# LUP-LuftbildUmweltPlanung/UNet

Hardware: AMD Instinct MI355X
Metric: 512x512 tiles/sec fwd+bwd (4-ch->5-class U-Net) (higher is better)
Workload: dtype f32

## Files before the change

### include/unet_hip.h

```cpp
#ifndef UNET_HIP_H
#define UNET_HIP_H

#include <stddef.h>
#include <stdint.h>

#ifdef __cplusplus
extern "C" {
#endif

#define UNET_OK 0
#define UNET_E_BADARG (-1)
#define UNET_E_UNSUPPORTED (-2)
#define UNET_E_HIP (-3)

#define UNET_ABI_VERSION 8

int unet_abi_version(void);
const char* unet_last_error(void);

#define UNET_F32 0
#define UNET_BF16 1
typedef uint16_t unet_bf16;

typedef struct {
    int conv_splitk;
    int mfma_shape;
    int f32_big_tile;
    int bf16_big_tile;
    int t256_tiles_per_wg;
    int t256_sliver;
    int conv1x1_gemm;
    int wgrad_mfma_shape;
    int wgrad_bf16_k4;
    int wgrad_1x1;
    int wgrad_narrow;
    int plan_batch;
    int wgrad_wgs;
    int conv_smallcin;
    int conv_head1x1;
} unet_tuning;
void unet_tuning_default(unet_tuning* t);


#define UNET_CONV_RELU 1
#define UNET_CONV_MASK 4

#define UNET_CONV_FWD 0
#define UNET_CONV_DGRAD 1

typedef struct {
    const float* x; int x_cs, x_co;
    const float* wp;
    const float* bias;
    const float* res; int res_cs, res_co;
    const float* mask; int mask_cs, mask_co;
    float* y; int y_cs, y_co;
    int N, IH, IW, Cin;
    int OH, OW, Cout;
    int ks, stride;
    int kind, flags;
    float* colsum;
    float* colsumsq;
    int cout_begin, cout_count;
    long long wp_img_stride;
    int dtype;
    int y_f32;
    float* splitk_ws;
    size_t splitk_ws_floats;
    const unet_tuning* tuning;
    int pixel_shuffle;
    const void* ps_tail;
    int ps_tail_cs, ps_tail_co;
    int ps_tail_c, ps_tail_at;
} unet_conv_desc;

int unet_conv2d_colsum_rows(const unet_conv_desc* d);
int unet_conv2d(const unet_conv_desc* d, void* stream);
size_t unet_conv2d_splitk_workspace(const unet_conv_desc* d);
int unet_conv2d_variant(const unet_conv_desc* d);
size_t unet_pack_weights_size(int Cout, int Cin, int ks, int mode);
int unet_pack_weights(const float* w, float* wp, int Cout, int Cin, int ks, int mode, void* stream);
int unet_pack_weights_strided(const float* w, long long so, long long sr, float* wp, int O, int R, void* stream);
size_t unet_pack_weights_size_bf16(int Cout, int Cin, int ks, int mode);
int unet_pack_weights_bf16(const float* w, unet_bf16* wp, int Cout, int Cin, int ks, int mode, void* stream);
typedef struct {
    const float* w;
    void* wp;
    int Cout, Cin, ks, mode;
    const float* out_scale;
} unet_pack_job;
size_t unet_pack_batch_table_bytes(int njobs);
int unet_pack_batch_build(const unet_pack_job* jobs, int njobs, int dtype, void* table_host, unsigned* total_blocks);
int unet_pack_batch_run(const void* table_dev, int njobs, unsigned total_blocks, int dtype, void* stream);
typedef struct {
    const float* x; int x_cs, x_co;
    const float* dy; int dy_cs, dy_co;
    float* dw;
    float* dbias;
    int N, IH, IW, Cin, OH, OW, Cout, ks, stride;
    float* workspace; size_t workspace_floats;
    int accumulate;
    int dtype;
    const unet_tuning* tuning;
} unet_wgrad_desc;
size_t unet_conv2d_wgrad_workspace(const unet_wgrad_desc* d);
int unet_conv2d_wgrad_dma(const unet_wgrad_desc* d);
int unet_conv2d_wgrad(const unet_wgrad_desc* d, void* stream);

int unet_bn_stats_rows(long long P);
int unet_bn_stats(const float* x, int x_cs, int x_co, long long P, int C, float* partial, void* stream);
int unet_bn_finalize(const float* psum, const float* psumsq, int rows, long long count, int C,
                     const float* gamma, const float* beta, float* running_mean, float* running_var,
                     float momentum, float eps,
                     float* scale, float* shift, float* save_mean, float* save_invstd, long long* batches_tracked, void* stream);
int unet_bn_eval_coeffs(const float* gamma, const float* beta, const float* running_mean, const float* running_var,
                        float eps, int C, float* scale, float* shift, void* stream);
int unet_affine_act(const float* x, int x_cs, int x_co, const float* scale, const float* shift,
                    const float* x2, int x2_cs, int x2_co, const float* scale2, const float* shift2,
                    float* y, int y_cs, int y_co, long long P, int C, int relu, void* stream);
int unet_bn_bwd_reduce(const float* dout, int d_cs, int d_co, const float* out, int o_cs, int o_co,
                       const float* x, int x_cs, int x_co, const float* mean, const float* invstd,
                       long long P, int C, float* partial, void* stream);
int unet_bn_bwd_finalize(const float* partial, int rows, long long count, int C,
                         float* dgamma, float* dbeta, float* c1, float* c2, void* stream);
int unet_bn_bwd_apply(const float* dout, int d_cs, int d_co, const float* out, int o_cs, int o_co,
                      const float* x, int x_cs, int x_co, const float* mean, const float* invstd,
                      const float* gamma, const float* c1, const float* c2,
                      float* dx, int dx_cs, int dx_co, float* gout, int g_cs, int g_co, int g_accumulate,
                      long long P, int C, void* stream);

int unet_maxpool3x3s2(const float* x, int x_cs, int x_co, float* y, int y_cs, int y_co, uint8_t* idx,
                      int N, int IH, int IW, int C, int OH, int OW, void* stream);
int unet_maxpool3x3s2_bwd(const float* dy, int dy_cs, int dy_co, const uint8_t* idx, float* dx, int dx_cs, int dx_co,
                          int N, int IH, int IW, int C, int OH, int OW, int accumulate, void* stream);
int unet_avgpool2_ceil(const float* x, int x_cs, int x_co, float* y, int y_cs, int y_co,
                       int N, int IH, int IW, int C, int OH, int OW, void* stream);
int unet_avgpool2_ceil_bwd(const float* dy, int dy_cs, int dy_co, float* dx, int dx_cs, int dx_co,
                           int N, int IH, int IW, int C, int OH, int OW, int accumulate, void* stream);

int unet_shuffle_blur(const float* yc, int yc_cs, int yc_co, float* X, int X_cs, int X_co,
                      int N, int h, int w, int Cu, int do_blur, void* stream);
int unet_shuffle_blur_bwd(const float* dX, int dX_cs, int dX_co, const float* yc, int yc_cs, int yc_co,
                          float* dyc, int dyc_cs, int dyc_co, int N, int h, int w, int Cu, int do_blur, void* stream);
int unet_shuffle_bwd_xmask(const float* dX, int dX_cs, int dX_co, const float* X, int X_cs, int X_co,
                           float* dyc, int dyc_cs, int dyc_co, int N, int h, int w, int Cu, void* stream);
int unet_resize_nearest(const float* x, int x_cs, int x_co, float* y, int y_cs, int y_co,
                        int N, int IH, int IW, int OH, int OW, int C, void* stream);
int unet_resize_nearest_bwd(const float* dy, int dy_cs, int dy_co, float* dx, int dx_cs, int dx_co,
                            int N, int IH, int IW, int OH, int OW, int C, void* stream);
int unet_nchw_to_nhwc(const float* x, float* y, int y_cs, int y_co, int N, int C, int H, int W, void* stream);
int unet_nhwc_to_nchw(const float* x, int x_cs, int x_co, float* y, int N, int C, int H, int W, void* stream);
int unet_copy_slice(const float* x, int x_cs, int x_co, float* y, int y_cs, int y_co, long long P, int C,
                    int accumulate, void* stream);
int unet_relu_mask(const float* g, int g_cs, int g_co, const float* ref, int r_cs, int r_co,
                   float* y, int y_cs, int y_co, long long P, int C, void* stream);
int unet_colsum(const float* x, int x_cs, int x_co, long long P, int C, float* out, float* workspace, void* stream);
size_t unet_colsum_workspace(long long P, int C);
int unet_dot(const float* x, int x_cs, int x_co, const float* y, int y_cs, int y_co, long long P, int C, float* out,
             float* workspace, void* stream);

size_t unet_ce_workspace(long long P);
int unet_ce_fwd(const float* z, int z_cs, int z_co, const int64_t* target, const float* weight, long long P, int C,
// ... 308 lines not shown
```

### unet_amd/csrc/conv1x1.hip

```cpp
#include "conv_common.h"

namespace {

typedef float f32x4 __attribute__((ext_vector_type(4)));
typedef __bf16 bf16x8 __attribute__((ext_vector_type(8)));
typedef __bf16 bf16x4 __attribute__((ext_vector_type(4)));
typedef unsigned short u16;

struct G1Args {
    const char* x; const char* wp; const float* bias; const char* res; const char* mask; char* y;
    int x_cs, x_co, res_cs, res_co, mask_cs, mask_co, y_cs, y_co;
    long long P;
    int nchunks, coutPad, n_base, n_end, Cout, relu, y_f32, ntn;
    long long ntiles;
    int ps, nf, H, W;
    const char* tail; int tail_cs, tail_co, tail_q, tail_at;
};

template <typename T, bool STAGED>
__global__ __launch_bounds__(256, 2) void conv1x1_gemm_kernel(const G1Args a) {
    constexpr int EB = (int)sizeof(T), KCB = 64;
    constexpr int MT = STAGED ? 8 : 4, NT = 4, TPIX = MT * 32, ROWB = 96, BUFB = TPIX * ROWB;
    extern __shared__ __attribute__((aligned(16))) char lds[];
    const int tid = threadIdx.x, lane = tid & 63, wave = __builtin_amdgcn_readfirstlane(tid >> 6);
    const int wm = wave >> 1, wn = wave & 1, l15 = lane & 15, kq = lane >> 4;
    const long long per_xcd = (long long)(gridDim.x >> 3);
    const long long wg = (long long)(blockIdx.x & 7) * per_xcd + (long long)(blockIdx.x >> 3);
    if (wg >= a.ntiles) return;
    const int nb = (int)(wg % a.ntn);
    const long long pt = wg / a.ntn;
    const long long p0 = pt * TPIX + wm * (TPIX / 2);
    const int c0 = a.n_base + nb * 128;

    const char* xp[MT];
#pragma unroll
    for (int m = 0; m < MT; ++m) {
        long long p = p0 + m * 16 + l15;
        p = p < a.P ? p : a.P - 1;
        xp[m] = a.x + ((size_t)p * a.x_cs + a.x_co) * EB + 16 * kq;
    }
    const char* wl = a.wp + ((size_t)(c0 + wn * 16 + l15) * KCB + 16 * kq);
    const size_t slab = (size_t)a.coutPad * KCB;
    int nv = 0;
#pragma unroll
    for (int n = 0; n < NT; ++n) nv += (c0 + (2 * n + wn) * 16 < a.n_end) ? 1 : 0;
    nv = __builtin_amdgcn_readfirstlane(nv);

    f32x4 acc[MT][NT];
#pragma unroll
    for (int m = 0; m < MT; ++m)
#pragma unroll
        for (int n = 0; n < NT; ++n) acc[m][n] = (f32x4){0.f, 0.f, 0.f, 0.f};

    auto mma = [&](const f32x4 (&xs)[MT], const f32x4 (&ws)[NT]) {
#pragma unroll
        for (int n = 0; n < NT; ++n) {
            if (n < nv) {
                if constexpr (EB == 2) {
                    const bf16x8 wv = __builtin_bit_cast(bf16x8, ws[n]);
#pragma unroll
                    for (int m = 0; m < MT; ++m)
                        acc[m][n] = __builtin_amdgcn_mfma_f32_16x16x32_bf16(wv, __builtin_bit_cast(bf16x8, xs[m]), acc[m][n], 0, 0, 0);
                } else {
#pragma unroll
                    for (int kk = 0; kk < 4; ++kk)
#pragma unroll
                        for (int m = 0; m < MT; ++m) acc[m][n] = __builtin_amdgcn_mfma_f32_16x16x4f32(ws[n][kk], xs[m][kk], acc[m][n], 0, 0, 0);
                }
            }
        }
    };
    const int last = a.nchunks - 1;
    if constexpr (!STAGED) {
        f32x4 xa[MT], wa[NT], xb[MT], wb[NT];
        auto load = [&](f32x4 (&xs)[MT], f32x4 (&ws)[NT], int c) {
#pragma unroll
            for (int m = 0; m < MT; ++m) xs[m] = *reinterpret_cast<const f32x4*>(xp[m] + (size_t)c * KCB);
#pragma unroll
            for (int n = 0; n < NT; ++n) ws[n] = *reinterpret_cast<const f32x4*>(wl + (size_t)c * slab + (size_t)n * 2048);
        };
        load(xa, wa, 0);
        for (int c = 0; c < a.nchunks; c += 2) {
            load(xb, wb, c + 1 < last ? c + 1 : last);
            mma(xa, wa);
            load(xa, wa, c + 2 < last ? c + 2 : last);
            if (c + 1 < a.nchunks) mma(xb, wb);
        }
    } else {
        const char* sp[4];
        unsigned so[4];
#pragma unroll
        for (int it = 0; it < 4; ++it) {
            const int e = tid + 256 * it, pe = e >> 2, q = e & 3;
            long long p = pt * TPIX + pe;
            p = p < a.P ? p : a.P - 1;
            sp[it] = a.x + ((size_t)p * a.x_cs + a.x_co) * EB + 16 * q;
            so[it] = (unsigned)(pe * ROWB + 16 * q);
        }
        const unsigned rbase = (unsigned)((wm * (TPIX / 2) + l15) * ROWB + 16 * kq);
// ... 25 lines not shown
            gload(wa, c + 2 < last ? c + 2 : last);
            if (c + 1 < a.nchunks) stage(wb, 1);
            sstore(0);
            __syncthreads();
        }
    }

    const T* resb = reinterpret_cast<const T*>(a.res);
    const T* maskb = reinterpret_cast<const T*>(a.mask);
    auto ld4 = [](const T* p_) -> f32x4 {
        if constexpr (EB == 2) {
            const uint2 u = *reinterpret_cast<const uint2*>(p_);
            return (f32x4){__uint_as_float(u.x << 16), __uint_as_float(u.x & 0xffff0000u), __uint_as_float(u.y << 16), __uint_as_float(u.y & 0xffff0000u)};
        } else return *reinterpret_cast<const f32x4*>(p_);
    };
    f32x4 bv[NT];
    int c4s[NT];
#pragma unroll
    for (int n = 0; n < NT; ++n) {
        const int c4 = c0 + (2 * n + wn) * 16 + 4 * kq;
        c4s[n] = c4;
        bv[n] = (f32x4){0.f, 0.f, 0.f, 0.f};
        if (a.bias != nullptr && n < nv && c4 < a.n_end) {
            if (a.ps) {
                const int ij = c4 / a.nf, c = c4 - ij * a.nf;
#pragma unroll
                for (int q = 0; q < 4; ++q) bv[n][q] = a.bias[4 * (c + q) + ij];
            } else {
#pragma unroll
                for (int q = 0; q < 4; ++q) bv[n][q] = (c4 + q < a.Cout) ? a.bias[c4 + q] : 0.f;
            }
        }
    }
#pragma unroll
    for (int m = 0; m < MT; ++m) {
        const long long p = p0 + m * 16 + l15;
        if (p >= a.P) continue;
        long long pimg = 0;
        int ph = 0, pw = 0;
        if (a.ps) {
            pimg = p / ((long long)a.H * a.W);
            const int rem = (int)(p - pimg * a.H * a.W);
            ph = rem / a.W; pw = rem - ph * a.W;
        }
#pragma unroll
        for (int n = 0; n < NT; ++n) {
            if (n >= nv) continue;
            const int c4 = c4s[n];
            if (c4 >= a.n_end) continue;
            f32x4 v = acc[m][n] + bv[n];
            if (resb != nullptr) v += ld4(resb + (size_t)p * a.res_cs + a.res_co + c4);
            if (a.relu) {
#pragma unroll
                for (int q = 0; q < 4; ++q) v[q] = fmaxf(v[q], 0.f);
            }
            if (maskb != nullptr) {
                const f32x4 mv = ld4(maskb + (size_t)p * a.mask_cs + a.mask_co + c4);
#pragma unroll
                for (int q = 0; q < 4; ++q) v[q] = mv[q] > 0.f ? v[q] : 0.f;
            }
            size_t yo = (size_t)p * a.y_cs + a.y_co + c4;
            if (a.ps) {
                const int ij = c4 / a.nf, c = c4 - ij * a.nf;
                yo = ((size_t)(pimg * 2 * a.H + 2 * ph + (ij >> 1)) * (2 * a.W) + 2 * pw + (ij & 1)) * a.y_cs + a.y_co + c;
            }
            if (EB == 4 || a.y_f32) *reinterpret_cast<f32x4*>(reinterpret_cast<float*>(a.y) + yo) = v;
            else {
                const bf16x4 o = {(__bf16)v[0], (__bf16)v[1], (__bf16)v[2], (__bf16)v[3]};
                *reinterpret_cast<uint2*>(reinterpret_cast<u16*>(a.y) + yo) = __builtin_bit_cast(uint2, o);
            }
            if (a.ps && a.tail != nullptr && c4 % a.nf == a.nf - 4) {
                const size_t op = (yo - (size_t)a.y_co - (size_t)(a.nf - 4)) / (size_t)a.y_cs;
                const char* src = a.tail + ((size_t)op * a.tail_cs + a.tail_co) * EB;
                char* dst = a.y + ((size_t)op * a.y_cs + a.tail_at) * EB;
                for (int t = 0; t < a.tail_q; ++t) {
                    if constexpr (EB == 4) *reinterpret_cast<f32x4*>(dst + 16 * t) = *reinterpret_cast<const f32x4*>(src + 16 * t);
                    else *reinterpret_cast<uint2*>(dst + 8 * t) = *reinterpret_cast<const uint2*>(src + 8 * t);
                }
            }
        }
    }
}


struct HeadArgs {
    const char* x; const char* wp; const float* bias; char* y;
    int x_cs, x_co, y_cs, y_co;
    long long P;
    int Cin, Cout, coutPad, relu, y_f32;
};

template <typename T, int NCH, int MT>
__global__ __launch_bounds__(256) void conv1x1_head_kernel(const HeadArgs a) {
    constexpr int EB = (int)sizeof(T), KC = 64 / EB, VEC = 16 / EB;
    const int lane = threadIdx.x & 63, l15 = lane & 15, kq = lane >> 4;
    const int nch = (a.Cin + KC - 1) / KC, tail = a.Cin % KC;
    const int cin_v = (a.Cin + VEC - 1) / VEC * VEC;
    f32x4 w[NCH];
#pragma unroll
    for (int c = 0; c < NCH; ++c) {
        w[c] = (f32x4){0.f, 0.f, 0.f, 0.f};
        if (c < nch) w[c] = *reinterpret_cast<const f32x4*>(a.wp + ((size_t)(c * a.coutPad + l15) * KC) * EB + 16 * kq);
    }
    float bv[4];
#pragma unroll
    for (int r = 0; r < 4; ++r) bv[r] = (a.bias != nullptr && 4 * kq + r < a.Cout) ? a.bias[4 * kq + r] : 0.f;
    const long long nwaves = (long long)gridDim.x * 4, wave0 = (long long)blockIdx.x * 4 + (threadIdx.x >> 6);
    constexpr int WP = 16 * MT;
    auto ldx = [](const char* q) { return *reinterpret_cast<const f32x4*>(q); };
    for (long long g = wave0; g * WP < a.P; g += nwaves) {
        f32x4 xs[MT][NCH];
        const char* xp[MT];
#pragma unroll
        for (int m = 0; m < MT; ++m) {
            long long p = g * WP + m * 16 + l15;
            p = p < a.P ? p : a.P - 1;
            xp[m] = a.x + ((size_t)p * a.x_cs + a.x_co) * EB;
#pragma unroll
            for (int c = 0; c < NCH; ++c) {
                xs[m][c] = (f32x4){0.f, 0.f, 0.f, 0.f};
                if constexpr (EB == 4) {
                    if (c < nch && !(tail != 0 && c == nch - 1)) xs[m][c] = ldx(xp[m] + (size_t)(c * KC + 4 * kq) * EB);
                    else if (c == nch - 1 && tail != 0) {
#pragma unroll
                        for (int kk = 0; kk < 4; ++kk)
                            if (kq + 4 * kk < tail) xs[m][c][kk] = *reinterpret_cast<const float*>(xp[m] + (size_t)(c * KC + kq + 4 * kk) * EB);
                    }
                } else {
                    if (c < nch && c * KC + VEC * kq < cin_v) xs[m][c] = ldx(xp[m] + (size_t)(c * KC + VEC * kq) * EB);
                }
            }
        }
        f32x4 acc[MT];
#pragma unroll
        for (int m = 0; m < MT; ++m) acc[m] = (f32x4){0.f, 0.f, 0.f, 0.f};
#pragma unroll
        for (int c = 0; c < NCH; ++c) {
            if (c < nch) {
                if constexpr (EB == 2) {
#pragma unroll
                    for (int m = 0; m < MT; ++m)
                        acc[m] = __builtin_amdgcn_mfma_f32_16x16x32_bf16(__builtin_bit_cast(bf16x8, w[c]), __builtin_bit_cast(bf16x8, xs[m][c]), acc[m], 0, 0, 0);
                } else {
                    const int steps = (tail != 0 && c == nch - 1) ? (tail + 3) / 4 : 4;
#pragma unroll
                    for (int kk = 0; kk < 4; ++kk)
                        if (kk < steps) {
#pragma unroll
                            for (int m = 0; m < MT; ++m) acc[m] = __builtin_amdgcn_mfma_f32_16x16x4f32(w[c][kk], xs[m][c][kk], acc[m], 0, 0, 0);
                        }
                }
            }
        }
        if (4 * kq < a.Cout) {
            const int nr = a.Cout - 4 * kq;
#pragma unroll
            for (int m = 0; m < MT; ++m) {
                const long long p = g * WP + m * 16 + l15;
                if (p >= a.P) continue;
                f32x4 v = acc[m];
#pragma unroll
                for (int r = 0; r < 4; ++r) {
                    v[r] += bv[r];
                    if (a.relu) v[r] = fmaxf(v[r], 0.f);
                }
                if (EB == 4 || a.y_f32) {
                    float* yo = reinterpret_cast<float*>(a.y) + (size_t)p * a.y_cs + a.y_co + 4 * kq;
                    if (nr >= 4) *reinterpret_cast<f32x4*>(yo) = v;
                    else {
#pragma unroll
                        for (int r = 0; r < 3; ++r) if (r < nr) yo[r] = v[r];
                    }
                } else {
                    __bf16* yo = reinterpret_cast<__bf16*>(a.y) + (size_t)p * a.y_cs + a.y_co + 4 * kq;
                    if (nr >= 4) *reinterpret_cast<bf16x4*>(yo) = (bf16x4){(__bf16)v[0], (__bf16)v[1], (__bf16)v[2], (__bf16)v[3]};
                    else {
#pragma unroll
                        for (int r = 0; r < 3; ++r) if (r < nr) yo[r] = (__bf16)v[r];
                    }
                }
            }
        }
    }
}
}

namespace unetconv {

static bool shape_ok(const unet_conv_desc* d) {
    if (d->ks != 1 || d->stride != 1 || d->wp_img_stride != 0 || d->colsum != nullptr || d->colsumsq != nullptr) return false;
    const int kct = d->dtype == UNET_BF16 ? 32 : 16;
    if (d->Cin < kct || d->Cin % kct != 0) return false;
    if (d->cout_begin % 128 != 0) return false;
    const int cols = d->cout_count ? d->cout_count : d->Cout;
    if (cols % 4 != 0 && d->cout_begin + cols != d->Cout) return false;
    const int pb = tuning_of(d->tuning).plan_batch;
    const long long P = (long long)(pb > 0 ? pb : d->N) * d->OH * d->OW;
    return ((P + 127) / 128) * ((cols + 127) / 128) >= 256;
}
static int form_of(const unet_conv_desc* d) {
    const int mode = tuning_of(d->tuning).conv1x1_gemm;
    if (d->pixel_shuffle) return mode == 1 ? 1 : 2;
    if (mode < 0) return 0;
    if (mode == 0) return d->dtype == UNET_BF16 ? 2 : 0;
    return mode == 1 ? 1 : 2;
}
bool conv_gemm1x1_applies(const unet_conv_desc* d) { return form_of(d) != 0 && shape_ok(d); }

int conv_gemm1x1_ps_check(const unet_conv_desc* d) {
    UNET_CHECK_ARG(d->x && d->wp && d->y && unet::aligned16(d->x) && unet::aligned16(d->wp) && unet::aligned16(d->y), "conv pixel_shuffle: null / unaligned tensor pointer");
    UNET_CHECK_ARG(d->dtype == UNET_F32 || d->dtype == UNET_BF16, "conv: unknown dtype %d", d->dtype);
    const int vec = d->dtype == UNET_BF16 ? 8 : 4;
    UNET_CHECK_ARG(d->ks == 1 && d->stride == 1 && d->kind == UNET_CONV_FWD && d->N > 0 && d->IH > 0 && d->IW > 0 && d->OH == d->IH && d->OW == d->IW && d->Cin > 0 && d->Cout > 0,
                   "conv pixel_shuffle: a 1x1 / stride-1 forward convolution");
    UNET_CHECK_ARG(d->Cout % 64 == 0, "conv pixel_shuffle: Cout = 4 nf with nf a multiple of 16 (got %d)", d->Cout);
    UNET_CHECK_ARG(unet::slice_ok_v(d->x_cs, d->x_co, d->Cin, vec), "conv pixel_shuffle: bad x slice");
    UNET_CHECK_ARG(unet::slice_ok_v(d->y_cs, d->y_co, d->Cout / 4, 4), "conv pixel_shuffle: bad y slice (Cout / 4 channels of a [N, 2 OH, 2 OW] tensor)");
    UNET_CHECK_ARG((d->flags & ~(UNET_CONV_RELU | UNET_CONV_MASK)) == 0, "conv pixel_shuffle: unknown flag bits 0x%x", d->flags);
    UNET_CHECK_ARG(d->bias == nullptr || (((uintptr_t)d->bias) & 3) == 0, "conv pixel_shuffle: bias must be a float pointer");
    UNET_CHECK_ARG(d->res == nullptr && !(d->flags & UNET_CONV_MASK) && d->colsum == nullptr && d->colsumsq == nullptr && d->cout_begin == 0 &&
                   d->cout_count == 0 && d->wp_img_stride == 0, "conv pixel_shuffle: no residual / mask / column sums / channel range / per-image filters");
    UNET_CHECK_ARG((long long)d->N * d->OH * d->OW * 4 < (1ll << 31), "conv pixel_shuffle: more than 2^31 output pixels");
    if (d->ps_tail != nullptr) {
        const int tq = unet::roundup(d->ps_tail_c, 4);
        UNET_CHECK_ARG(unet::aligned16(d->ps_tail) && d->ps_tail_c > 0 && d->ps_tail_cs > 0 && d->ps_tail_cs % 4 == 0 && d->ps_tail_co >= 0 && d->ps_tail_co % 4 == 0 &&
                       d->ps_tail_co + tq <= d->ps_tail_cs, "conv pixel_shuffle: bad ps_tail slice (whole quads: cs, co multiples of 4, co + roundup(c, 4) <= cs)");
        UNET_CHECK_ARG(d->ps_tail_at % 4 == 0 && d->ps_tail_at >= d->y_co + d->Cout / 4 && d->ps_tail_at + tq <= d->y_cs && !(d->dtype == UNET_BF16 && d->y_f32),
                       "conv pixel_shuffle: ps_tail_at must be a multiple of 4 behind the shuffled channels with ps_tail_at + roundup(ps_tail_c, 4) <= y_cs");
    }
    if (!shape_ok(d)) {
        unet::set_error("conv pixel_shuffle: only conv1x1_gemm_kernel stores pixel-shuffled (whole reduction chunks, >= 256 blocks of 128 x 128); "
                        "ask unet_conv2d_variant first and keep conv + unet_shuffle_blur otherwise");
        return UNET_E_UNSUPPORTED;
    }
    return UNET_OK;
}

int conv_gemm1x1(const unet_conv_desc* d, hipStream_t st) {
    G1Args a;
    const bool bf = d->dtype == UNET_BF16;
    const int kct = bf ? 32 : 16;
    a.x = (const char*)d->x; a.wp = (const char*)d->wp; a.bias = d->bias; a.res = (const char*)d->res;
    a.mask = (d->flags & UNET_CONV_MASK) ? (const char*)d->mask : nullptr; a.y = (char*)d->y;
    a.x_cs = d->x_cs; a.x_co = d->x_co; a.res_cs = d->res_cs; a.res_co = d->res_co; a.mask_cs = d->mask_cs; a.mask_co = d->mask_co;
    a.y_cs = d->y_cs; a.y_co = d->y_co;
    a.P = (long long)d->N * d->OH * d->OW;
    a.nchunks = d->Cin / kct;
    a.coutPad = unet::roundup(d->Cout, 128);
    a.n_base = d->cout_begin;
    a.n_end = d->cout_begin + (d->cout_count ? d->cout_count : d->Cout);
    a.Cout = d->Cout;
    a.relu = (d->flags & UNET_CONV_RELU) ? 1 : 0;
    a.y_f32 = bf ? d->y_f32 : 1;
    a.tail = d->pixel_shuffle ? (const char*)d->ps_tail : nullptr;
    a.tail_cs = d->ps_tail_cs; a.tail_co = d->ps_tail_co; a.tail_q = unet::roundup(d->ps_tail_c, 4) / 4; a.tail_at = d->ps_tail_at;
    const bool staged = form_of(d) == 2;
    const int tpix = staged ? 256 : 128;
    a.ntn = unet::cdiv(a.n_end - a.n_base, 128);
    a.ntiles = ((a.P + tpix - 1) / tpix) * a.ntn;
    a.ps = d->pixel_shuffle ? 1 : 0; a.nf = d->Cout / 4; a.H = d->OH; a.W = d->OW;
    UNET_CHECK_ARG(a.ntiles < (1ll << 31) - 8, "conv 1x1: grid too large");
    const unsigned grid = (unsigned)((a.ntiles + 7) / 8 * 8);
    if (staged) {
        if (bf) hipLaunchKernelGGL((conv1x1_gemm_kernel<unsigned short, true>), dim3(grid), dim3(256), 2 * 256 * 96, st, a);
        else hipLaunchKernelGGL((conv1x1_gemm_kernel<float, true>), dim3(grid), dim3(256), 2 * 256 * 96, st, a);
    } else {
        if (bf) hipLaunchKernelGGL((conv1x1_gemm_kernel<unsigned short, false>), dim3(grid), dim3(256), 0, st, a);
        else hipLaunchKernelGGL((conv1x1_gemm_kernel<float, false>), dim3(grid), dim3(256), 0, st, a);
    }
    UNET_CHECK_LAUNCH();
    return UNET_OK;
}


bool conv_head1x1_applies(const unet_conv_desc* d) {
    if (tuning_of(d->tuning).conv_head1x1 == 0) return false;
    const int vec = d->dtype == UNET_BF16 ? 8 : 4;
    return d->ks == 1 && d->stride == 1 && d->Cin > 8 && d->Cin <= 128 && d->Cout <= 16 && d->res == nullptr && !(d->flags & UNET_CONV_MASK) &&
           d->colsum == nullptr && d->colsumsq == nullptr && d->cout_begin == 0 && (d->cout_count == 0 || d->cout_count == d->Cout) &&
           d->wp_img_stride == 0 && !d->pixel_shuffle && unet::roundup(d->Cin, vec) <= d->x_cs - d->x_co && d->Cout <= d->y_cs - d->y_co &&
           d->y_co % 4 == 0 && d->y_cs % 4 == 0 && d->x_co % vec == 0 && d->x_cs % vec == 0;
}

int conv_head1x1(const unet_conv_desc* d, hipStream_t st) {
    HeadArgs a;
    const bool bf = d->dtype == UNET_BF16;
    a.x = (const char*)d->x; a.wp = (const char*)d->wp; a.bias = d->bias; a.y = (char*)d->y;
    a.x_cs = d->x_cs; a.x_co = d->x_co; a.y_cs = d->y_cs; a.y_co = d->y_co;
    a.P = (long long)d->N * d->OH * d->OW;
    a.Cin = d->Cin; a.Cout = d->Cout; a.coutPad = unet::roundup(d->Cout, 128);
    a.relu = (d->flags & UNET_CONV_RELU) ? 1 : 0;
    a.y_f32 = bf ? d->y_f32 : 1;
    const bool swap = tuning_of(d->tuning).conv_head1x1 == 2;
    const int mt = (bf != swap) ? 4 : 2;
    long long blocks = (a.P + 64 * mt - 1) / (64 * mt);
    if (blocks > 256 * 16) blocks = 256 * 16;
    void (*kern)(const HeadArgs);
    if (bf) kern = mt == 4 ? conv1x1_head_kernel<u16, 4, 4> : conv1x1_head_kernel<u16, 4, 2>;
    else kern = mt == 4 ? conv1x1_head_kernel<float, 8, 4> : conv1x1_head_kernel<float, 8, 2>;
    hipLaunchKernelGGL(kern, dim3((unsigned)blocks), dim3(256), 0, st, a);
    UNET_CHECK_LAUNCH();
    return UNET_OK;
}

}
```

### unet_amd/csrc/conv_common.h

```cpp
#pragma once
#include "common.h"

namespace unetconv {

constexpr int KC = 16;
constexpr int LDK = 20;
constexpr int KCB = 32;
constexpr int LDKB = 24;

struct TapSet {
    int n;
    int min_dy, min_dx;
    int ext_y, ext_x;
    int py, px;
    signed char dy[9], dx[9], widx[9];
    unsigned long long dpack, wpack;
};

struct KArgs {
    const float* x; const float* wp; const float* bias; const float* res; const float* mask;
    float* y; float* colsum; float* colsumsq;
    int x_cs, x_co, res_cs, res_co, mask_cs, mask_co, y_cs, y_co;
    int N, IH, IW, Cin, Cin4;
    int OH, OW, Cout;
// ... 148 lines not shown
__device__ __forceinline__ void wait_loads(v4f (&b)[NB], v4f (&h)[NH]) {
    static_assert((NB == 2 || NB == 4) && (NH == 4 || NH == 6 || NH == 10), "register groups");
#define UNET_H4 "+v"(h[0]), "+v"(h[1]), "+v"(h[2]), "+v"(h[3])
#define UNET_H6 UNET_H4, "+v"(h[4]), "+v"(h[5])
#define UNET_H10 UNET_H4, "+v"(h[4]), "+v"(h[5]), "+v"(h[6]), "+v"(h[7]), "+v"(h[8]), "+v"(h[9])
    if constexpr (NB == 4 && NH == 6) asm volatile("s_waitcnt vmcnt(0)" : "+v"(b[0]), "+v"(b[1]), "+v"(b[2]), "+v"(b[3]), UNET_H6);
    else if constexpr (NB == 2 && NH == 6) asm volatile("s_waitcnt vmcnt(0)" : "+v"(b[0]), "+v"(b[1]), UNET_H6);
    else if constexpr (NB == 2 && NH == 4) asm volatile("s_waitcnt vmcnt(0)" : "+v"(b[0]), "+v"(b[1]), UNET_H4);
    else if constexpr (NB == 2) asm volatile("s_waitcnt vmcnt(0)" : "+v"(b[0]), "+v"(b[1]), UNET_H10);
    else if constexpr (NH == 4) asm volatile("s_waitcnt vmcnt(0)" : "+v"(b[0]), "+v"(b[1]), "+v"(b[2]), "+v"(b[3]), UNET_H4);
    else asm volatile("s_waitcnt vmcnt(0)" : "+v"(b[0]), "+v"(b[1]), "+v"(b[2]), "+v"(b[3]), UNET_H10);
#undef UNET_H4
#undef UNET_H6
#undef UNET_H10
}

struct Plan {
    KArgs k;
    int tw, bm, bn, hit, nparity, mf, max_hpix;
    size_t lds_bytes;
    dim3 grid;
    int splits, cp;
    size_t ws_floats;
    unet_tuning tune;
};


__device__ __forceinline__ float ld_act(const float* p) { return *p; }
__device__ __forceinline__ float ld_act(const unsigned short* p) { return __uint_as_float((unsigned)*p << 16); }
__device__ __forceinline__ void st_act(float* p, float v) { *p = v; }
__device__ __forceinline__ void st_act(unsigned short* p, float v) { *p = __builtin_bit_cast(unsigned short, (__bf16)v); }

template <auto Kern, typename... Args>
int launch_big_lds(dim3 grid, dim3 block, size_t lds_bytes, hipStream_t st, const Args&... args) {
    static unsigned long long configured = 0;
    if (unet::first_use_on_device(&configured))
        UNET_CHECK_HIP(hipFuncSetAttribute((const void*)Kern, hipFuncAttributeMaxDynamicSharedMemorySize, 160 * 1024));
    hipLaunchKernelGGL(Kern, grid, block, lds_bytes, st, args...);
    UNET_CHECK_LAUNCH();
    return UNET_OK;
}

template <typename K, int TW, int HIT>
int launch_bn(const Plan& p, int y_f32, hipStream_t st) {
    if (p.bm == 64) {
        if (p.bn == 64) return K::template launch<TW, 1, 1, 2, 2, HIT>(p, y_f32, st);
        return K::template launch<TW, 1, 2, 2, 2, HIT>(p, y_f32, st);
    }
    switch (p.bn) {
        case 32: return K::template launch<TW, 1, 1, 4, 1, HIT>(p, y_f32, st);
        case 64: return K::template launch<TW, 2, 1, 2, 2, HIT>(p, y_f32, st);
        default: return K::template launch<TW, 2, 2, 2, 2, HIT>(p, y_f32, st);
    }
}
template <typename K, int HIT>
int launch_tw(const Plan& p, int y_f32, hipStream_t st) {
    switch (p.tw) {
        case 32: return launch_bn<K, 32, HIT>(p, y_f32, st);
        case 16: return launch_bn<K, 16, HIT>(p, y_f32, st);
        default: return launch_bn<K, 8, HIT>(p, y_f32, st);
    }
}
template <typename K>
int launch_generic(const Plan& p, int y_f32, hipStream_t st) {
    if (p.bm == 256 || p.hit == 6) {
        unet::set_error("conv: inconsistent plan (the 256-pixel tile / halo item count 6 on the generic kernels)");
        return UNET_E_UNSUPPORTED;
    }
    return p.hit == 10 ? launch_tw<K, 10>(p, y_f32, st) : launch_tw<K, 4>(p, y_f32, st);
}

int conv_generic_f32(const Plan& p, hipStream_t st);
int conv_generic_bf16(const Plan& p, int y_f32, hipStream_t st);
int conv_t256(const Plan& p, int dtype, int y_f32, hipStream_t st);
int splitk_reduce(const unet_conv_desc* d, const Plan& p, hipStream_t st);
bool conv_smallk_applies(const unet_conv_desc* d);
int conv_smallk(const unet_conv_desc* d, hipStream_t st);
bool conv_smallcin_applies(const unet_conv_desc* d);
int conv_smallcin(const unet_conv_desc* d, hipStream_t st);
bool conv_head1x1_applies(const unet_conv_desc* d);
int conv_head1x1(const unet_conv_desc* d, hipStream_t st);
bool conv_gemm1x1_applies(const unet_conv_desc* d);
int conv_gemm1x1(const unet_conv_desc* d, hipStream_t st);
int conv_gemm1x1_ps_check(const unet_conv_desc* d);

}
```

### unet_amd/csrc/conv_dispatch.hip

```cpp
#include <stdlib.h>

#include "conv_common.h"

namespace unetconv {
static int env_int(const char* name, int dflt) {
    const char* e = getenv(name);
    return (e != nullptr && e[0] != 0) ? atoi(e) : dflt;
}
const unet_tuning& tuning_defaults() {
    static const unet_tuning t = [] {
        unet_tuning v;
        v.conv_splitk = env_int("UNET_CONV_SPLITK", 1);
        v.mfma_shape = 16;
        v.f32_big_tile = 1;
        v.bf16_big_tile = 1;
        v.t256_tiles_per_wg = 0;
        v.t256_sliver = env_int("UNET_T256_SLIVER", 1);
        v.conv1x1_gemm = env_int("UNET_CONV1X1_GEMM", 0);
        v.wgrad_mfma_shape = 32;
        v.wgrad_bf16_k4 = 1;
        v.wgrad_1x1 = 1;
        v.wgrad_narrow = 1;
        v.plan_batch = 0;
        v.wgrad_wgs = env_int("UNET_WGRAD_WGS", 0);
        v.conv_smallcin = env_int("UNET_CONV_SMALLCIN", 1);
        v.conv_head1x1 = env_int("UNET_CONV_HEAD1X1", 1);
        return v;
    }();
    return t;
}
}

extern "C" void unet_tuning_default(unet_tuning* t) {
    if (t != nullptr) *t = unetconv::tuning_defaults();
}

namespace {

using namespace unetconv;

int make_plan(const unet_conv_desc* d, Plan* p, int kc, int vec, int mf, int big_tile, int splitk, int plan_batch) {
    UNET_CHECK_ARG(d != nullptr, "conv: null desc");
    UNET_CHECK_ARG(d->x && d->wp && d->y, "conv: null tensor pointer");
    UNET_CHECK_ARG(d->ks == 1 || d->ks == 3, "conv: ks must be 1 or 3 (got %d)", d->ks);
    UNET_CHECK_ARG(d->stride == 1 || d->stride == 2, "conv: stride must be 1 or 2 (got %d)", d->stride);
    UNET_CHECK_ARG(!(d->ks == 1 && d->stride != 1), "conv: 1x1 stride 2 unsupported");
    UNET_CHECK_ARG(d->N > 0 && d->IH > 0 && d->IW > 0 && d->OH > 0 && d->OW > 0 && d->Cin > 0 && d->Cout > 0, "conv: bad dims");
    UNET_CHECK_ARG(unet::slice_ok_v(d->x_cs, d->x_co, d->Cin, vec), "conv: bad x slice cs=%d co=%d C=%d", d->x_cs, d->x_co, d->Cin);
    UNET_CHECK_ARG(unet::slice_ok_v(d->y_cs, d->y_co, d->Cout, d->y_f32 ? 4 : vec), "conv: bad y slice cs=%d co=%d C=%d", d->y_cs, d->y_co, d->Cout);
    UNET_CHECK_ARG(unet::aligned16(d->x) && unet::aligned16(d->wp), "conv: x/wp must be 16-byte aligned");
    if (d->res) UNET_CHECK_ARG(unet::slice_ok_v(d->res_cs, d->res_co, d->Cout, vec), "conv: bad res slice");
    if (d->flags & UNET_CONV_MASK) UNET_CHECK_ARG(d->mask && unet::slice_ok_v(d->mask_cs, d->mask_co, d->Cout, vec), "conv: bad mask slice");
    const int pad = (d->ks - 1) / 2;
    if (d->kind == UNET_CONV_FWD) {
        UNET_CHECK_ARG(d->OH == (d->IH + 2 * pad - d->ks) / d->stride + 1 && d->OW == (d->IW + 2 * pad - d->ks) / d->stride + 1,
                       "conv fwd: output dims %dx%d inconsistent with input %dx%d ks %d stride %d", d->OH, d->OW, d->IH, d->IW, d->ks, d->stride);
    } else if (d->kind == UNET_CONV_DGRAD) {
        UNET_CHECK_ARG(d->IH == (d->OH + 2 * pad - d->ks) / d->stride + 1 && d->IW == (d->OW + 2 * pad - d->ks) / d->stride + 1,
                       "conv dgrad: grad dims %dx%d inconsistent with input dims %dx%d", d->IH, d->IW, d->OH, d->OW);
    } else {
        UNET_CHECK_ARG(false, "conv: bad kind %d", d->kind);
    }
    UNET_CHECK_ARG((long long)d->IH * d->IW * d->x_cs < (1ll << 31) && (long long)d->OH * d->OW * d->y_cs < (1ll << 31) &&
                       (long long)d->OH * d->OW * (d->res ? d->res_cs : 1) < (1ll << 31) &&
                       (long long)d->OH * d->OW * ((d->flags & UNET_CONV_MASK) ? d->mask_cs : 1) < (1ll << 31),
                   "conv: image too large for 32-bit in-image offsets");

    KArgs& k = p->k;
    memset(&k, 0, sizeof(k));
    k.x = d->x; k.wp = d->wp; k.bias = d->bias; k.res = d->res; k.mask = (d->flags & UNET_CONV_MASK) ? d->mask : nullptr;
    k.y = d->y; k.colsum = d->colsum; k.colsumsq = d->colsumsq;
    k.x_cs = d->x_cs; k.x_co = d->x_co; k.res_cs = d->res_cs; k.res_co = d->res_co;
    k.mask_cs = d->mask_cs; k.mask_co = d->mask_co; k.y_cs = d->y_cs; k.y_co = d->y_co;
    k.N = d->N; k.IH = d->IH; k.IW = d->IW; k.Cin = d->Cin; k.Cin4 = unet::roundup(d->Cin, vec);
    k.OH = d->OH; k.OW = d->OW; k.Cout = d->Cout;
    const int cols = d->cout_count > 0 ? d->cout_count : d->Cout;
    UNET_CHECK_ARG(d->cout_begin >= 0 && (d->cout_begin & 15) == 0 && d->cout_begin + cols <= d->Cout, "conv: bad cout range [%d,+%d) of %d",
                   d->cout_begin, cols, d->Cout);
    k.n_base = d->cout_begin; k.n_end = d->cout_begin + cols;
    UNET_CHECK_ARG(d->wp_img_stride >= 0 && (d->wp_img_stride & 3) == 0, "conv: bad wp_img_stride");
    k.wp_stride = d->wp_img_stride;
    k.flags = d->flags;
    k.nchunks = unet::cdiv(d->Cin, kc);
    k.coutPad = unet::roundup(d->Cout, 128);
    p->nparity = 1;
    k.S = 1; k.OS = 1; k.TSH = d->OH; k.TSW = d->OW;

    const int T = d->ks * d->ks;
    if (d->kind == UNET_CONV_FWD) {
        k.S = d->stride;
        TapSet& t = k.taps[0];
        t.n = T; t.min_dy = -pad; t.min_dx = -pad; t.ext_y = d->ks; t.ext_x = d->ks; t.py = t.px = 0;
        for (int r = 0; r < d->ks; ++r)
            for (int s = 0; s < d->ks; ++s) {
                const int i = r * d->ks + s;
                t.dy[i] = (signed char)(r - pad); t.dx[i] = (signed char)(s - pad); t.widx[i] = (signed char)i;
            }
    } else if (d->stride == 1) {
        TapSet& t = k.taps[0];
        t.n = T; t.min_dy = -pad; t.min_dx = -pad; t.ext_y = d->ks; t.ext_x = d->ks; t.py = t.px = 0;
        for (int r = 0; r < d->ks; ++r)
            for (int s = 0; s < d->ks; ++s) {
                const int i = r * d->ks + s;
                t.dy[i] = (signed char)(pad - r); t.dx[i] = (signed char)(pad - s); t.widx[i] = (signed char)i;
            }
    } else {
        k.OS = 2; k.TSH = (d->OH + 1) / 2; k.TSW = (d->OW + 1) / 2;
        p->nparity = 4;
        for (int py = 0; py < 2; ++py)
            for (int px = 0; px < 2; ++px) {
                TapSet& t = k.taps[py * 2 + px];
                int rs[2], rdy[2], nr, ss[2], sdx[2], ns;
// ... 118 lines not shown
    UNET_CHECK_ARG(t.mfma_shape == 16 || t.mfma_shape == 32, "conv: unet_tuning.mfma_shape must be 16 or 32 (start from unet_tuning_default())");
    const int rc = make_plan(d, p, KC, 4, t.mfma_shape, t.f32_big_tile ? 1 : 0, splitk < 0 ? t.conv_splitk : splitk, t.plan_batch);
    p->tune = t;
    return rc;
}
int plan_bf16(const unet_conv_desc* d, Plan* p, int splitk = -1) {
    UNET_CHECK_ARG(d != nullptr, "conv: null desc");
    const unet_tuning t = tuning_of(d->tuning);
    int rc = make_plan(d, p, KCB, 8, 16, t.bf16_big_tile, splitk < 0 ? t.conv_splitk : splitk, t.plan_batch);
    p->tune = t;
    if (rc != UNET_OK) return rc;
    UNET_CHECK_ARG(d->colsum == nullptr && d->colsumsq == nullptr, "conv bf16: column sums are not available in the bf16 kernel");
    p->lds_bytes = (size_t)(32 + 2 * p->max_hpix * LDKB) * sizeof(float);
    p->k.fold = (p->nparity == 1 && p->splits == 1 && bf16_fold_tail(d->Cin, d->ks * d->ks)) ? 1 : 0;
    UNET_CHECK_ARG(d->Cout % 4 == 0 || d->y_co + unet::roundup(d->Cout, 4) <= d->y_cs, "conv bf16: the output slice must own its 4-channel padding");
    UNET_CHECK_ARG(unet::aligned16(d->y) && (!d->res || unet::aligned16(d->res)) && (!d->mask || unet::aligned16(d->mask)),
                   "conv bf16: y/res/mask must be 16-byte aligned");
    return UNET_OK;
}
int plan(const unet_conv_desc* d, Plan* p, int splitk = -1) {
    return d != nullptr && d->dtype == UNET_BF16 ? plan_bf16(d, p, splitk) : plan_f32(d, p, splitk);
}

enum class Family { PixelShuffle, SmallK, SmallCin, Head1x1, Gemm1x1, T256, Generic };

int choose(const unet_conv_desc* d, Family* f, Plan* p) {
    if (d != nullptr && d->pixel_shuffle) {
        *f = Family::PixelShuffle;
        return conv_gemm1x1_ps_check(d);
    }
    int rc = plan(d, p);
    if (rc == UNET_OK && !splitk_redirect(d, p)) rc = plan(d, p, 0);
    if (rc != UNET_OK) return rc;
    if (conv_smallk_applies(d)) *f = Family::SmallK;
    else if (conv_smallcin_applies(d)) *f = Family::SmallCin;
    else if (conv_head1x1_applies(d)) *f = Family::Head1x1;
    else if (conv_gemm1x1_applies(d)) *f = Family::Gemm1x1;
    else *f = p->hit == 6 ? Family::T256 : Family::Generic;
    return UNET_OK;
}

int variant_id(Family f, const Plan& p) {
    switch (f) {
        case Family::PixelShuffle: case Family::Gemm1x1: return 8;
        case Family::SmallK: return 9;
        case Family::SmallCin: return 10;
        case Family::Head1x1: return 11;
        default: break;
    }
    const bool large = p.bm == 256 && p.bn == 128 && p.tw == 32 && (long long)p.k.mtiles * p.k.ntn >= 512;
    return p.tw * 10000 + p.bn * 10 + (p.hit == 10 ? 1 : 0) + (p.bm == 64 ? 5 : 0) + (p.bm == 256 ? (large ? 7 : 6) : 0) + (p.splits > 1 ? 1000000 * p.splits : 0);
}

}

extern "C" int unet_conv2d(const unet_conv_desc* d, void* stream) {
    UNET_CHECK_ARG(d == nullptr || d->pixel_shuffle || d->dtype == UNET_F32 || d->dtype == UNET_BF16, "conv: unknown dtype %d", d->dtype);
    Family f;
    Plan p;
    int rc = choose(d, &f, &p);
    if (rc != UNET_OK) return rc;
    hipStream_t st = (hipStream_t)stream;
    const bool bf = d->dtype == UNET_BF16;
    const int y_f32 = p.splits > 1 ? 1 : d->y_f32;
    switch (f) {
        case Family::PixelShuffle: case Family::Gemm1x1: return conv_gemm1x1(d, st);
        case Family::SmallK: return conv_smallk(d, st);
        case Family::SmallCin: return conv_smallcin(d, st);
        case Family::Head1x1: return conv_head1x1(d, st);
        case Family::T256: rc = conv_t256(p, d->dtype, y_f32, st); break;
        case Family::Generic: rc = bf ? conv_generic_bf16(p, y_f32, st) : conv_generic_f32(p, st); break;
    }
    if (rc != UNET_OK || p.splits <= 1) return rc;
    return splitk_reduce(d, p, st);
}

extern "C" int unet_conv2d_variant(const unet_conv_desc* d) {
    Family f;
    Plan p;
    const int rc = choose(d, &f, &p);
    return rc == UNET_OK ? variant_id(f, p) : rc;
}

extern "C" size_t unet_conv2d_splitk_workspace(const unet_conv_desc* d) {
    Plan p;
    if (d == nullptr || d->pixel_shuffle) return 0;
    return plan(d, &p) == UNET_OK ? p.ws_floats : 0;
}

extern "C" int unet_conv2d_colsum_rows(const unet_conv_desc* d) {
    Plan p;
    const int rc = plan_f32(d, &p, 0);
    if (rc != UNET_OK) return rc;
    const int wm = (p.bn == 32 && p.bm == 128) ? 4 : 2;
    return p.nparity * p.k.mtiles * wm;
}
```

Baseline: 150.4.

## Add ring-buffered 1x1 conv GEMM kernel with direct buffer-to-LDS loads

Adds an f32 1x1-conv GEMM kernel that streams activation chunks straight into a double-buffered, swizzled LDS ring via buffer_load_lds. Each workgroup walks several consecutive pixel tiles, prefetching the next stage while computing the current one and keeping weights in registers. The kernel becomes the default for pixel-shuffle convs and for wide f32 forward 1x1 convs. The goal is to hide global-load latency and amortize per-workgroup setup, at the cost of more LDS, a specialised path, and heuristic dispatch thresholds.

Result: no change. 150.5, median of 3 (+0.1%).

```diff
diff --git a/include/unet_hip.h b/include/unet_hip.h
--- a/include/unet_hip.h
+++ b/include/unet_hip.h
@@ -78,6 +78,7 @@
 int unet_conv2d(const unet_conv_desc* d, void* stream);
 size_t unet_conv2d_splitk_workspace(const unet_conv_desc* d);
 int unet_conv2d_variant(const unet_conv_desc* d);
+int unet_conv1x1_form(const unet_conv_desc* d);
 size_t unet_pack_weights_size(int Cout, int Cin, int ks, int mode);
 int unet_pack_weights(const float* w, float* wp, int Cout, int Cin, int ks, int mode, void* stream);
 int unet_pack_weights_strided(const float* w, long long so, long long sr, float* wp, int O, int R, void* stream);
diff --git a/unet_amd/csrc/conv1x1.hip b/unet_amd/csrc/conv1x1.hip
--- a/unet_amd/csrc/conv1x1.hip
+++ b/unet_amd/csrc/conv1x1.hip
@@ -1,3 +1,5 @@
+#include <type_traits>
+
 #include "conv_common.h"
 
 namespace {
@@ -15,6 +17,7 @@
     long long ntiles;
     int ps, nf, H, W;
     const char* tail; int tail_cs, tail_co, tail_q, tail_at;
+    int tpw; long long nptiles;
 };
 
 template <typename T, bool STAGED>
@@ -206,6 +209,180 @@
     }
 }
 
+__global__ __launch_bounds__(256, 2) void conv1x1_ring_kernel(const G1Args a) {
+    constexpr int KCB = 64, MT = 8, NT = 4, TPIX = 256, SLOTB = TPIX * KCB;
+    typedef __attribute__((address_space(3))) void* lds_ptr;
+    extern __shared__ __attribute__((aligned(16))) char lds[];
+    const int tid = threadIdx.x, lane = tid & 63, wave = __builtin_amdgcn_readfirstlane(tid >> 6);
+    const int wm = wave >> 1, wn = wave & 1, l15 = lane & 15, kq = lane >> 4;
+    const long long per_xcd = (long long)(gridDim.x >> 3);
+    const long long wg = (long long)(blockIdx.x & 7) * per_xcd + (long long)(blockIdx.x >> 3);
+    if (wg >= a.ntiles) return;
+    const int nb = (int)(wg % a.ntn);
+    const long long t0 = (wg / a.ntn) * a.tpw;
+    const int nt = (int)(a.nptiles - t0 < a.tpw ? a.nptiles - t0 : a.tpw);
+    const int c0 = a.n_base + nb * 128;
+    const int np = (a.nchunks + 1) >> 1, nstages = nt * np;
+
+    const char* wl = a.wp + ((size_t)(c0 + wn * 16 + l15) * KCB + 16 * kq);
+    const size_t slab = (size_t)a.coutPad * KCB;
+    int nv = 0;
+#pragma unroll
+    for (int n = 0; n < NT; ++n) nv += (c0 + (2 * n + wn) * 16 < a.n_end) ? 1 : 0;
+    nv = __builtin_amdgcn_readfirstlane(nv);
+
+    unsigned vo[4];
+#pragma unroll
+    for (int it = 0; it < 4; ++it) {
+        const int e = tid + 256 * it, pe = e >> 2;
+        vo[it] = (unsigned)pe * (unsigned)a.x_cs * 4u + 16u * (unsigned)((e & 3) ^ ((-(pe >> 2)) & 3));
+    }
+    const unsigned rbase = (unsigned)((wm * (TPIX / 2) + l15) * KCB + 16 * (kq ^ ((-(l15 >> 2)) & 3)));
+
+    f32x4 acc[MT][NT];
+    auto zero_acc = [&]() {
+#pragma unroll
+        for (int m = 0; m < MT; ++m)
+#pragma unroll
+            for (int n = 0; n < NT; ++n) acc[m][n] = (f32x4){0.f, 0.f, 0.f, 0.f};
+    };
+    zero_acc();
+
+    int dt = 0, dk = 0, ds = 0;
+    auto dma_stage = [&]() {
+        const long long tp = (t0 + dt) * TPIX;
+        const long long left = a.P - tp;
+        const int npix = left < TPIX ? (int)left : TPIX;
+        const __amdgpu_buffer_rsrc_t rs = __builtin_amdgcn_make_buffer_rsrc(
+            const_cast<char*>(a.x) + ((size_t)tp * a.x_cs + a.x_co) * 4, 0, ((npix - 1) * a.x_cs + a.nchunks * 16) * 4, 0x00020000);
+        char* dst = lds + (ds & 1) * 2 * SLOTB + wave * 1024;
+#pragma unroll
+        for (int ch = 0; ch < 2; ++ch) {
+            const int c = 2 * dk + ch;
+            if (c < a.nchunks) {
+#pragma unroll
+                for (int it = 0; it < 4; ++it)
+                    __builtin_amdgcn_raw_ptr_buffer_load_lds(rs, (lds_ptr)(dst + ch * SLOTB + it * 4096), 16, (int)(vo[it] + (unsigned)c * KCB), 0, 0, 0);
+            }
+        }
+        ++ds;
+        if (++dk == np) { dk = 0; ++dt; }
+    };
+    auto wload = [&](f32x4 (&ws)[NT], int c) {
+#pragma unroll
+        for (int n = 0; n < NT; ++n) ws[n] = *reinterpret_cast<const f32x4*>(wl + (size_t)c * slab + (size_t)n * 2048);
+    };
+    auto xread = [&](f32x4 (&xs)[MT], const char* slot) {
+#pragma unroll
+        for (int m = 0; m < MT; ++m) xs[m] = *reinterpret_cast<const f32x4*>(slot + rbase + m * 16 * KCB);
+    };
+
+    const float* resb = reinterpret_cast<const float*>(a.res);
+    const float* maskb = reinterpret_cast<const float*>(a.mask);
+    f32x4 bv[NT];
+    int c4s[NT];
+    float* const bias_lds = reinterpret_cast<float*>(lds + 4 * SLOTB);
+    if (tid < 128) {
+        const int ch = c0 + tid;
+        float b = 0.f;
+        if (a.bias != nullptr && ch < a.n_end && ch < a.Cout) b = a.ps ? a.bias[4 * (ch % a.nf) + ch / a.nf] : a.bias[ch];
+        bias_lds[tid] = b;
+    }
+    auto load_bias = [&]() {
+#pragma unroll
+        for (int n = 0; n < NT; ++n) {
+            c4s[n] = c0 + (2 * n + wn) * 16 + 4 * kq;
+            bv[n] = *reinterpret_cast<const f32x4*>(bias_lds + (2 * n + wn) * 16 + 4 * kq);
+        }
+    };
+    auto store_row = [&](auto nvc, int m, long long p) {
+        constexpr int NV = decltype(nvc)::value;
+        if (p >= a.P) return;
+        long long pimg = 0;
+        int ph = 0, pw = 0;
+        if (a.ps) {
+            pimg = p / ((long long)a.H * a.W);
+            const int rem = (int)(p - pimg * a.H * a.W);
+            ph = rem / a.W; pw = rem - ph * a.W;
+        }
+#pragma unroll
+        for (int n = 0; n < NT; ++n) {
+            if (n >= NV) continue;
+            const int c4 = c4s[n];
+            if (c4 >= a.n_end) continue;
+            f32x4 v = acc[m][n] + bv[n];
+            if (resb != nullptr) v += *reinterpret_cast<const f32x4*>(resb + (size_t)p * a.res_cs + a.res_co + c4);
+            if (a.relu) {
+#pragma unroll
+                for (int q = 0; q < 4; ++q) v[q] = fmaxf(v[q], 0.f);
+            }
+            if (maskb != nullptr) {
+                const f32x4 mv = *reinterpret_cast<const f32x4*>(maskb + (size_t)p * a.mask_cs + a.mask_co + c4);
+#pragma unroll
+                for (int q = 0; q < 4; ++q) v[q] = mv[q] > 0.f ? v[q] : 0.f;
+            }
+            size_t yo = (size_t)p * a.y_cs + a.y_co + c4;
+            if (a.ps) {
+                const int ij = c4 / a.nf, c = c4 - ij * a.nf;
+                yo = ((size_t)(pimg * 2 * a.H + 2 * ph + (ij >> 1)) * (2 * a.W) + 2 * pw + (ij & 1)) * a.y_cs + a.y_co + c;
+            }
+            *reinterpret_cast<f32x4*>(reinterpret_cast<float*>(a.y) + yo) = v;
+            if (a.ps && a.tail != nullptr && c4 % a.nf == a.nf - 4) {
+                const size_t op = (yo - (size_t)a.y_co - (size_t)(a.nf - 4)) / (size_t)a.y_cs;
+                const char* src = a.tail + ((size_t)op * a.tail_cs + a.tail_co) * 4;
+                char* dst = a.y + ((size_t)op * a.y_cs + a.tail_at) * 4;
+                for (int t = 0; t < a.tail_q; ++t) *reinterpret_cast<f32x4*>(dst + 16 * t) = *reinterpret_cast<const f32x4*>(src + 16 * t);
+            }
+        }
+    };
+    auto run = [&](auto nvc) {
+    constexpr int NV = decltype(nvc)::value;
+    f32x4 wc[NT], wx[NT];
+    dma_stage();
+    wload(wc, 0);
+    int c = 0, ct = 0, s = 0;
+    for (;;) {
+        const bool first = (c & 1) == 0, lastc = c == a.nchunks - 1;
+        if (first) asm volatile("s_waitcnt vmcnt(0) lgkmcnt(0)\n\ts_barrier" : "+v"(wc[0]), "+v"(wc[1]), "+v"(wc[2]), "+v"(wc[3]) : : "memory");
+        f32x4 xs[MT];
+        xread(xs, lds + ((s & 1) * 2 + (c & 1)) * SLOTB);
+        if (first && s + 1 < nstages) dma_stage();
+        wload(wx, lastc ? 0 : c + 1);
+        const long long p0 = (t0 + ct) * TPIX + wm * (TPIX / 2);
+        if (lastc) load_bias();
+#pragma unroll
+        for (int m = 0; m < MT; ++m) {
+#pragma unroll
+            for (int kk = 0; kk < 4; ++kk)
+#pragma unroll
+                for (int n = 0; n < NT; ++n)
+                    if (n < NV) acc[m][n] = __builtin_amdgcn_mfma_f32_16x16x4f32(wc[n][kk], xs[m][kk], acc[m][n], 0, 0, 0);
+            if (lastc) {
+                store_row(nvc, m, p0 + m * 16 + l15);
+#pragma unroll
+                for (int n = 0; n < NT; ++n) acc[m][n] = (f32x4){0.f, 0.f, 0.f, 0.f};
+            }
+        }
+#pragma unroll
+        for (int n = 0; n < NT; ++n) wc[n] = wx[n];
+        if (lastc) {
+            c = 0; ++s;
+            if (++ct == nt) break;
+        } else {
+            ++c;
+            s += (c & 1) ? 0 : 1;
+        }
+    }
+    };
+    switch (nv) {
+        case 4: run(std::integral_constant<int, 4>()); break;
+        case 3: run(std::integral_constant<int, 3>()); break;
+        case 2: run(std::integral_constant<int, 2>()); break;
+        case 1: run(std::integral_constant<int, 1>()); break;
+        default: run(std::integral_constant<int, 0>()); break;
+    }
+}
+
 
 struct HeadArgs {
     const char* x; const char* wp; const float* bias; char* y;
@@ -324,12 +501,14 @@
 }
 static int form_of(const unet_conv_desc* d) {
     const int mode = tuning_of(d->tuning).conv1x1_gemm;
-    if (d->pixel_shuffle) return mode == 1 ? 1 : 2;
+    const int wide = (mode == 3 && d->dtype != UNET_BF16) ? 3 : 2;
+    if (d->pixel_shuffle) return mode == 1 ? 1 : (mode == 0 && conv1x1_ring_default(d) ? 3 : wide);
     if (mode < 0) return 0;
-    if (mode == 0) return d->dtype == UNET_BF16 ? 2 : 0;
-    return mode == 1 ? 1 : 2;
+    if (mode == 0) return d->dtype == UNET_BF16 ? 2 : (conv1x1_ring_default(d) ? 3 : 0);
+    return mode == 1 ? 1 : wide;
 }
 bool conv_gemm1x1_applies(const unet_conv_desc* d) { return form_of(d) != 0 && shape_ok(d); }
+int conv_gemm1x1_form(const unet_conv_desc* d) { return shape_ok(d) ? form_of(d) : 0; }
 
 int conv_gemm1x1_ps_check(const unet_conv_desc* d) {
     UNET_CHECK_ARG(d->x && d->wp && d->y && unet::aligned16(d->x) && unet::aligned16(d->wp) && unet::aligned16(d->y), "conv pixel_shuffle: null / unaligned tensor pointer");
@@ -378,14 +557,22 @@
     a.y_f32 = bf ? d->y_f32 : 1;
     a.tail = d->pixel_shuffle ? (const char*)d->ps_tail : nullptr;
     a.tail_cs = d->ps_tail_cs; a.tail_co = d->ps_tail_co; a.tail_q = unet::roundup(d->ps_tail_c, 4) / 4; a.tail_at = d->ps_tail_at;
-    const bool staged = form_of(d) == 2;
+    const int form = form_of(d);
+    const bool staged = form >= 2;
     const int tpix = staged ? 256 : 128;
     a.ntn = unet::cdiv(a.n_end - a.n_base, 128);
-    a.ntiles = ((a.P + tpix - 1) / tpix) * a.ntn;
+    a.nptiles = (a.P + tpix - 1) / tpix;
+    const int pb = tuning_of(d->tuning).plan_batch;
+    const long long walk = (((long long)(pb > 0 ? pb : d->N) * d->OH * d->OW + tpix - 1) / tpix) * a.ntn / 2048;
+    a.tpw = form == 3 ? (int)(walk < 1 ? 1 : (walk > 4 ? 4 : walk)) : 1;
+    a.ntiles = ((a.nptiles + a.tpw - 1) / a.tpw) * a.ntn;
     a.ps = d->pixel_shuffle ? 1 : 0; a.nf = d->Cout / 4; a.H = d->OH; a.W = d->OW;
     UNET_CHECK_ARG(a.ntiles < (1ll << 31) - 8, "conv 1x1: grid too large");
     const unsigned grid = (unsigned)((a.ntiles + 7) / 8 * 8);
-    if (staged) {
+    if (form == 3) {
+        UNET_CHECK_ARG(255ll * d->x_cs + d->Cin < (1ll << 28), "conv 1x1: pixel stride too large for the ring form");
+        return launch_big_lds<conv1x1_ring_kernel>(dim3(grid), dim3(256), 4 * 256 * 64 + 128 * 4, st, a);
+    } else if (staged) {
         if (bf) hipLaunchKernelGGL((conv1x1_gemm_kernel<unsigned short, true>), dim3(grid), dim3(256), 2 * 256 * 96, st, a);
         else hipLaunchKernelGGL((conv1x1_gemm_kernel<float, true>), dim3(grid), dim3(256), 2 * 256 * 96, st, a);
     } else {
diff --git a/unet_amd/csrc/conv_common.h b/unet_amd/csrc/conv_common.h
--- a/unet_amd/csrc/conv_common.h
+++ b/unet_amd/csrc/conv_common.h
@@ -254,6 +254,8 @@
 int conv_head1x1(const unet_conv_desc* d, hipStream_t st);
 bool conv_gemm1x1_applies(const unet_conv_desc* d);
 int conv_gemm1x1(const unet_conv_desc* d, hipStream_t st);
+int conv_gemm1x1_form(const unet_conv_desc* d);
+bool conv1x1_ring_default(const unet_conv_desc* d);
 int conv_gemm1x1_ps_check(const unet_conv_desc* d);
 
 }
diff --git a/unet_amd/csrc/conv_dispatch.hip b/unet_amd/csrc/conv_dispatch.hip
--- a/unet_amd/csrc/conv_dispatch.hip
+++ b/unet_amd/csrc/conv_dispatch.hip
@@ -28,6 +28,16 @@
         return v;
     }();
     return t;
+}
+
+bool conv1x1_ring_default(const unet_conv_desc* d) {
+    if (d->dtype == UNET_BF16) return false;
+    if (d->pixel_shuffle) return true;
+    if (d->kind != UNET_CONV_FWD) return false;
+    const int cols = d->cout_count ? d->cout_count : d->Cout;
+    const int pb = tuning_of(d->tuning).plan_batch;
+    const long long P = (long long)(pb > 0 ? pb : d->N) * d->OH * d->OW;
+    return d->Cin >= 96 && d->Cin <= 512 && cols % 128 == 0 && cols >= 384 && cols >= 2 * d->Cin && ((P + 255) / 256) * (cols / 128) >= 512;
 }
 }
 
@@ -312,6 +322,14 @@
     return rc == UNET_OK ? variant_id(f, p) : rc;
 }
 
+extern "C" int unet_conv1x1_form(const unet_conv_desc* d) {
+    Family f;
+    Plan p;
+    const int rc = choose(d, &f, &p);
+    if (rc != UNET_OK) return rc;
+    return (f == Family::PixelShuffle || f == Family::Gemm1x1) ? conv_gemm1x1_form(d) : 0;
+}
+
 extern "C" size_t unet_conv2d_splitk_workspace(const unet_conv_desc* d) {
     Plan p;
     if (d == nullptr || d->pixel_shuffle) return 0;
```
